# M4THYOU/TokenDagger

Hardware: AMD Instinct MI355X
Metric: GB/s raw text tokenized (Llama-4 vocab, 1024 MB corpus) (higher is better)
Workload: dtype u8

## Files before the change

### include/tokendagger_hip.h

```cpp
#ifndef TOKENDAGGER_HIP_H
#define TOKENDAGGER_HIP_H

#include <stdint.h>

#ifdef __cplusplus
extern "C" {
#endif

#define TD_OK 0
#define TD_E_INVALID 1
#define TD_E_PATTERN 2
#define TD_E_VOCAB 3
#define TD_E_UNKNOWN_BYTE 4
#define TD_E_CAPACITY 5
#define TD_E_SCRATCH 6
#define TD_E_HIP 7
#define TD_E_BAD_TOKEN 8
#define TD_E_SPECIAL 9

#define TD_MODE_ENCODE 0
#define TD_MODE_ORDINARY 1

typedef struct td_tokenizer td_tokenizer;

// ... 36 lines not shown
                                      const uint8_t* allowed_bytes, const int64_t* allowed_offsets, int64_t n_allowed,
                                      int32_t* out_tokens, int64_t out_capacity, int64_t* out_offsets, int64_t* n_tokens);

#define TD_INFO_N_PAIRS 1
#define TD_INFO_MERGE_CLOSED 2
#define TD_INFO_MAX_ID 3
#define TD_INFO_TILE_BYTES 4
#define TD_INFO_WORKSPACE_BYTES 5
#define TD_INFO_N_SPECIAL 6
#define TD_INFO_LONG_PIECES 7
#define TD_INFO_FAR_PIECES 8
#define TD_INFO_DEFERRED_TILES 9
#define TD_INFO_FLAGGED_TILES 10
#define TD_INFO_LB_TIMEOUTS 12
#define TD_INFO_REPEATS 13
#define TD_INFO_LISTED_PIECES 14
#define TD_INFO_CHAR_SEEDS 15
#define TD_INFO_SPARSE 16
#define TD_INFO_WS_FILLED_BYTES 17
#define TD_INFO_SMALL_ENCODES 18
#define TD_INFO_SMALL_ENCODE_HANDBACKS 19
#define TD_INFO_SMALL_DECODES 20
#define TD_INFO_SMALL_DECODE_HANDBACKS 21
#define TD_INFO_DIRECT_TILES 11
int64_t td_info(const td_tokenizer* t, int what);

int td_encode_device_with_special(td_tokenizer* t, const void* d_text, int64_t n_bytes, const void* d_doc_offsets, int64_t n_docs,
                                  const int32_t* allowed_ids, int64_t n_allowed, void* d_out_tokens, int64_t out_capacity,
                                  void* d_out_offsets, void* hip_stream);

#define TD_UNIT_BYTES 0
#define TD_UNIT_CHARS 1

int td_token_starts(td_tokenizer* t, const int32_t* tokens, int64_t n_tokens, const int64_t* tok_offsets, int64_t n_docs, int unit,
                    int64_t* out_starts);
int td_token_starts_device(td_tokenizer* t, const void* d_tokens, int64_t n_tokens, const void* d_tok_offsets, int64_t n_docs, int unit,
                           void* d_out_starts, void* hip_stream);

int td_encode_batch_with_starts(td_tokenizer* t, const uint8_t* text, const int64_t* doc_offsets, int64_t n_docs, int mode,
                                const uint8_t* allowed_bytes, const int64_t* allowed_offsets, int64_t n_allowed, int unit,
                                int32_t* out_tokens, int64_t out_capacity, int64_t* out_offsets, int64_t* out_starts, int64_t* n_tokens);

int td_encode_device_with_starts(td_tokenizer* t, const void* d_text, int64_t n_bytes, const void* d_doc_offsets, int64_t n_docs, int mode,
                                 int unit, void* d_out_tokens, int64_t out_capacity, void* d_out_offsets, void* d_out_starts,
                                 void* hip_stream);

// ... 425 lines not shown
```

### tokendagger_amd/capi.py

```python
from __future__ import annotations

import ctypes
from pathlib import Path

import numpy as np

_PKG = Path(__file__).resolve().parent
LIB_PATH = _PKG / "libtokendagger_hip.so"

TD_OK = 0
TD_E_CAPACITY = 5
TD_MODE_ENCODE = 0
TD_MODE_ORDINARY = 1
TD_E_INVALID = 1
TD_E_BAD_TOKEN = 8
TD_UNIT_BYTES, TD_UNIT_CHARS = 0, 1
TD_ROWS_CONCAT, TD_ROWS_PAD, TD_ROWS_BESTFIT, TD_ROWS_WINDOWS = 0, 1, 2, 3
TD_ROWS_DROP_LAST = 1
TD_ROWS_TRUNCATE = 2
TD_INFO_N_PAIRS, TD_INFO_MERGE_CLOSED, TD_INFO_MAX_ID, TD_INFO_TILE_BYTES = 1, 2, 3, 4
TD_INFO_WORKSPACE_BYTES, TD_INFO_N_SPECIAL, TD_INFO_LONG_PIECES, TD_INFO_FAR_PIECES = 5, 6, 7, 8
TD_OPT_LONG_POOL_BYTES = 1
TD_OPT_PROFILE = 2
TD_OPT_PIPE_CHUNK_BYTES = 3
# ... 4 lines not shown
TD_OPT_DEVICE_SPECIALS = 8
TD_OPT_DIRECT = 9
TD_OPT_PACK_SPLIT = 10
TD_OPT_DEDUPE = 11
TD_OPT_OVERLAP = 12
TD_OPT_GIANT_COOP_MIN = 13
TD_OPT_SPARSE = 14
TD_OPT_COUNTS_SEATS = 15
TD_OPT_COUNTS_FLUSH_TILES = 16
TD_COUNTS_ACCUMULATE = 1
TD_OPT_NGRAM_TAG_BITS = 17
TD_NGRAM_ACCUMULATE = 1
TD_NGRAM_MAX_LEN, TD_NGRAM_MAX_LENGTHS = 64, 8
TD_MINHASH_MAX_PERM = 1024
TD_NGRAM_INFO = {"patterns": 1, "distinct": 2, "lengths": 3, "max_len": 4, "slots": 5, "max_probe": 6, "device_bytes": 7}
TD_INFO_DEFERRED_TILES, TD_INFO_FLAGGED_TILES = 9, 10
TD_INFO_DIRECT_TILES = 11
TD_INFO_LB_TIMEOUTS = 12
TD_INFO_REPEATS, TD_INFO_LISTED_PIECES, TD_INFO_CHAR_SEEDS = 13, 14, 15
TD_INFO_SPARSE = 16
TD_OPT_WS_FILL = 18
TD_INFO_WS_FILLED_BYTES = 17
TD_INFO_SMALL_ENCODES, TD_INFO_SMALL_ENCODE_HANDBACKS, TD_INFO_SMALL_DECODES, TD_INFO_SMALL_DECODE_HANDBACKS = 18, 19, 20, 21

EXPORTS = [
    "td_create", "td_clone", "td_destroy", "td_last_error", "td_encode_batch", "td_encode_device", "td_reserve",
    "td_device_status", "td_decode_bytes", "td_encode_with_special", "td_info", "td_set_option",
    "td_special_count", "td_special_get", "td_profile_read",
    "td_vocab_create", "td_vocab_destroy", "td_vocab_error", "td_vocab_load_tiktoken", "td_vocab_load_hf_special",
    "td_vocab_load_tekken", "td_vocab_load_json", "td_vocab_set_pattern", "td_vocab_pattern", "td_vocab_arrays",
    "td_create_from_vocab", "td_token_bytes", "td_single_token", "td_decode_device", "td_decode_batch", "td_encode_batch_with_special",
    "td_encode_with_special_strs", "td_encode_batch_with_special_strs", "td_profile_read_ex", "td_profile_segment_name",
    "td_comm_unique_id", "td_comm_create", "td_comm_destroy", "td_comm_gather_counts", "td_comm_bases", "td_comm_gather_tokens",
    "td_comm_last_error", "td_encode_device_with_special", "td_token_starts", "td_token_starts_device", "td_encode_batch_with_starts",
    "td_encode_device_with_starts", "td_make_rows_device", "td_make_rows", "td_encode_batch_rows",
    "td_pack_plan", "td_pack_rows", "td_pack_rows_device", "td_encode_batch_pack_rows",
    "td_window_plan", "td_window_rows", "td_window_rows_device", "td_encode_batch_window_rows",
    "td_span_labels", "td_span_labels_device", "td_encode_batch_span_labels",
    "td_make_rows_labeled", "td_make_rows_labeled_device", "td_pack_rows_labeled", "td_pack_rows_labeled_device",
    "td_window_rows_labeled", "td_window_rows_labeled_device", "td_encode_batch_span_label_rows",
    "td_select_plan", "td_select_docs", "td_select_docs_device", "td_encode_batch_select",
    "td_join_plan", "td_join_fields", "td_join_fields_device", "td_encode_batch_join",
    "td_range_plan", "td_range_labels", "td_range_labels_device", "td_encode_batch_range_labels", "td_encode_batch_range_label_rows",
    "td_token_counts_host", "td_token_counts", "td_token_counts_device", "td_encode_batch_token_counts",
    "td_decode_rows_check", "td_decode_rows", "td_decode_rows_device",
    "td_ngram_set_create", "td_ngram_set_destroy", "td_ngram_set_info", "td_ngram_matches_host", "td_ngram_matches_device",
# ... 1967 lines not shown
```

### tokendagger_amd/csrc/td_api.cpp

```cpp
#include "td_counts_args.h"
#include "td_handle.h"
#include "td_regex.h"

static thread_local std::string g_create_err;
static thread_local std::string g_thread_err;
static thread_local const td_tokenizer* g_thread_err_owner = nullptr;

namespace td {

hipError_t make_stream(Stream& s) {
    hipStream_t h = nullptr;
    const hipError_t e = hipStreamCreateWithFlags(&h, hipStreamNonBlocking);
    if (e == hipSuccess) s = Stream(h);
    return e;
}
hipError_t make_event(Event& ev) {
    hipEvent_t h = nullptr;
    const hipError_t e = hipEventCreateWithFlags(&h, hipEventDisableTiming);
    if (e == hipSuccess) ev = Event(h);
    return e;
}
hipError_t make_pinned(PinnedBuf& b, size_t bytes) {
    void* p = nullptr;
    const hipError_t e = hipHostMalloc(&p, bytes, hipHostMallocDefault);
// ... 311 lines not shown
    a.dd_table = a.dedupe ? (unsigned long long*)t->dd_table.p : nullptr;
    a.dd_mask = a.dedupe ? dd_entries(t, n) - 1u : 0u;
    a.flagged_count = &ctl->flagged_count;
    a.rx = t->d_rx;
    a.rx_stage1 = t->d_rx_s1;
    a.rx_stage2 = t->d_rx_s2;
    a.gap_list = (int64_t*)t->gap_list.p;
    a.gap_cap = (uint32_t)std::min<size_t>(t->gap_list.cap / 4, 0x7FFFFFF0u);
    a.gapbits = (uint32_t*)t->gapbits.p;
    a.gx_chunk = gx_chunk_for(n);
    a.gx_exit = (int64_t*)t->gx_exit.p;
    a.gx_state = (uint32_t*)t->gx_state.p;
    a.gap_count = &ctl->gap_count;
    a.gx_prefix = t->gx_prefix_dev;
    a.flagged_list = (uint32_t*)t->flagged_list.p;
    a.deferred_list = (uint32_t*)t->deferred_list.p;
    a.deferred_count = &ctl->deferred_count;
    a.fused = t->opt.fused ? 1 : 0;
    a.pack_split = t->opt.pack_split ? 1 : 0;
    a.direct = (t->opt.direct && t->opt.fused && !t->sp_active && t->H.pattern_kind != PATTERN_GENERIC && d_out && !t->stop_after) ? 1 : 0;
    a.tile_state = (unsigned long long*)t->tile_state.p;
    a.slab = (uint32_t*)t->slab.p;
    a.direct_tiles = &ctl->direct_tiles;
    a.probe_deferred = 0;
    a.miss_cap = (uint32_t)((n_tiles + 1) * K_MISS_LISTED_MAX);
    a.chunk_pref = (int64_t*)t->chunk_pref.p;
    a.ctl_reset = &ctl->long_count;
    a.ctl_reset_words = (uint32_t)((sizeof(Ctl) - offsetof(Ctl, long_count)) / 4);
    a.out_tokens = (int32_t*)d_out;
    a.out_cap = d_out ? out_cap : 0;
    a.out_offsets = (int64_t*)d_out_offs;
    a.err = &ctl->err;
    a.err_pos = &ctl->err_pos;
    a.n_tiles = (int)n_tiles;
    a.n_stiles = (int)((n + KS_TILE - 1) / KS_TILE);
    a.pat_flags = pattern_flags(t->H.pattern_kind);
    a.use_fastpath = (mode == TD_MODE_ENCODE) || t->H.merge_closed;
    a.text_aligned = (((uintptr_t)d_text) & 15) == 0;
    a.stop_after = t->stop_after;
    if (t->sp_active) {
        a.sp.bytes = (const uint8_t*)t->sp_bytes.p;
        a.sp.off = (const uint32_t*)t->sp_off.p;
        a.sp.len = (const uint32_t*)t->sp_len.p;
        a.sp.id = (const int32_t*)t->sp_id.p;
        a.sp.parent = (const int32_t*)t->sp_parent.p;
        a.sp.first2 = (const uint32_t*)t->sp_first2.p;
// ... 82 lines not shown
            return "No value found for piece at byte offset " + std::to_string(pos) + ": byte sequence is not in the vocabulary";
        case TD_E_CAPACITY:
            return "output capacity too small: " + std::to_string(pos) + (rows_last ? " rows needed" : " tokens needed");
        case TD_E_BAD_TOKEN:
            return "Invalid token for decoding at index " + std::to_string(pos);
        case TD_E_SCRATCH:
            return "device scratch exhausted near byte offset " + std::to_string(pos) +
                   " (pieces above 64 bytes: raise TD_OPT_LONG_POOL_BYTES; allowed special tokens: more candidates than one per 32 bytes of the batch)";
    }
    return "device error " + std::to_string(code) + " at byte offset " + std::to_string(pos);
}

int td::absorb_ctl(td_tokenizer* t, Ctl c, hipStream_t stream, int64_t* err_pos) {
    int rc0;
    if (c.err == TD_E_BAD_TOKEN) c.err_pos = 0x7FFFFFFFFFFFFFFFll - c.err_pos;
    t->last_long = c.long_count;
    t->last_far = (int64_t)c.slow_count + c.far_tiles;
    t->last_giant = c.giant_count;
    t->seen_counters = true;
    t->last_deferred = c.deferred_count;
    t->last_flagged = c.flagged_count;
    t->last_direct = c.direct_tiles;
    t->last_timeouts = c.lb_timeouts;
    t->last_repeats = c.dd_stats[0];
    t->last_listed = c.dd_stats[1];
    if (err_pos) *err_pos = c.err_pos;
    if (c.err != 0) {
        if ((rc0 = zero_wait(t, t->ctl.p, sizeof(Ctl), stream))) return rc0;
        t->err = device_error_text(c.err, c.err_pos, t->rows_last);
        return c.err;
    }
    return TD_OK;
}

int td::device_status_locked(td_tokenizer* t, hipStream_t stream, int64_t* err_pos) {
    if (!t->ctl.p) { HIP_TRY(t, hipStreamSynchronize(stream)); return TD_OK; }
    int rc0 = own_streams(t);
    if (rc0) return rc0;
    static_assert(sizeof(Ctl) <= 256, "h_ctl");
    HIP_TRY(t, hipMemcpyAsync(t->h_ctl.p, t->ctl.p, sizeof(Ctl), hipMemcpyDeviceToHost, stream));
    HIP_TRY(t, hipStreamSynchronize(stream));
    if (!t->has_last || t->last_stream == stream) t->graveyard.clear();
    return absorb_ctl(t, *(const Ctl*)t->h_ctl.p, stream, err_pos);
}

namespace {
// ... 14 lines not shown
    t->s_h2d = std::move(h2d);
    return TD_OK;
}

int encode_batch_pipelined(td_tokenizer* t, const uint8_t* text, const int64_t* doc_offsets, int64_t n_docs, int mode,
                           int32_t* out_tokens, int64_t out_capacity, int64_t* out_offsets, int64_t* n_tokens) {
    int rc;
    if ((rc = pipe_init(t))) return rc;
    if (!t->pool_threads || t->pool_threads->size() != std::max(t->opt.pipe_threads - 1, 1)) t->pool_threads.reset(new CopyPool(std::max(t->opt.pipe_threads - 1, 1)));
    if ((rc = order_before(t, t->s_k))) return rc;
    const int64_t n_all = doc_offsets[n_docs] - doc_offsets[0];
    const int64_t chunk_bytes = std::min(t->opt.pipe_chunk_bytes, std::max<int64_t>(t->opt.pipe_chunk_bytes / 8, n_all / 6));
    std::vector<int64_t> cd{0};
    for (int64_t d = 0; d < n_docs;) {
        const int64_t lo = doc_offsets[d];
        int64_t e = d + 1;
        int64_t a = d + 1, b = n_docs;
        while (a < b) { const int64_t mid = (a + b + 1) >> 1; if (doc_offsets[mid] - lo <= chunk_bytes) a = mid; else b = mid - 1; }
        e = std::max(e, a);
        cd.push_back(e);
        d = e;
    }
    const int nchunks = (int)cd.size() - 1;
    t->last_direct = t->last_timeouts = 0;
    struct Pending { int64_t d0, d1, b0, nbytes, ntok; };
    std::vector<Pending> pend((size_t)nchunks);
    int64_t tok_base = 0;
    bool capacity_miss = false;
    int first_err = TD_OK;
    constexpr int NS = td_tokenizer::PIPE_SLOTS;
    const bool timing = getenv("TD_PIPE_TIMING") != nullptr;
    static const bool publish = !(getenv("TD_PIPE_PUBLISH") && atoi(getenv("TD_PIPE_PUBLISH")) == 0);
    static const int d2h_blocks = getenv("TD_PIPE_D2H_KERNEL") ? atoi(getenv("TD_PIPE_D2H_KERNEL")) : 32;
    double tm[6] = {0, 0, 0, 0, 0, 0};
    auto now = [] { return std::chrono::steady_clock::now(); };
    auto lap = [&](int k, std::chrono::steady_clock::time_point t0) { if (timing) tm[k] += std::chrono::duration<double, std::milli>(now() - t0).count(); };
    std::shared_ptr<CopyPool::Job> in_job[NS], out_job[NS];
    auto start_in = [&](int i) -> int {
        td_tokenizer::PipeSlot& sl = t->pipe[i % NS];
        const int64_t d0 = cd[(size_t)i], d1 = cd[(size_t)i + 1], b0 = doc_offsets[d0], nb = doc_offsets[d1] - b0;
        const auto t0 = now();
        int r;
        if ((r = pinned_ensure(t, sl.h_text, (size_t)nb + 64))) return r;
        in_job[i % NS] = t->pool_threads->copy(sl.h_text.p, text + b0, (size_t)nb);
        lap(5, t0);
        return TD_OK;
    };
// ... 22 lines not shown
        if ((r = encode_device_locked(t, sl.d_text.p, nb, sl.d_offs.p, nd, mode, sl.d_tok.p, std::max<int64_t>(nb, 1), sl.d_toff.p, t->s_k))) return r;
        if (publish) {
            HIP_TRY(t, launch_pipe_publish(t->ctl.p, (uint32_t)sizeof(Ctl), sl.h_ctl.p, (const int64_t*)sl.d_toff.p, nd + 1, (int64_t*)sl.h_offs.p, t->s_k));
        } else {
            HIP_TRY(t, hipMemcpyAsync(sl.h_ctl.p, t->ctl.p, sizeof(Ctl), hipMemcpyDeviceToHost, t->s_k));
            HIP_TRY(t, hipMemcpyAsync(sl.h_offs.p, sl.d_toff.p, (size_t)(nd + 1) * 8, hipMemcpyDeviceToHost, t->s_k));
        }
        HIP_TRY(t, hipEventRecord(sl.ev_off, t->s_k));
        lap(1, t0);
        return TD_OK;
    };
    auto fetch = [&](int i) -> int {
        td_tokenizer::PipeSlot& sl = t->pipe[i % NS];
        Pending& P = pend[(size_t)i];
        auto t0 = now();
        HIP_TRY(t, hipEventSynchronize(sl.ev_off));
        lap(2, t0);
        const int64_t nd = P.d1 - P.d0;
        const int64_t* to = (const int64_t*)sl.h_offs.p;
        const Ctl& c = *(const Ctl*)sl.h_ctl.p;
        P.ntok = to[nd];
        t->last_direct += c.direct_tiles;
        t->last_timeouts += c.lb_timeouts;
        if (c.err != 0 && first_err == TD_OK) {
            first_err = c.err;
            const long long pos = c.err_pos + (first_err == TD_E_UNKNOWN_BYTE || first_err == TD_E_SCRATCH ? P.b0 : 0);
            t->err = first_err == TD_E_UNKNOWN_BYTE ? device_error_text(first_err, pos, false)
                                                    : "device error " + std::to_string(first_err) + " near byte offset " + std::to_string(pos);
        }
        for (int64_t k = 0; k < nd; ++k) out_offsets[P.d0 + k] = tok_base + to[k];
        if (tok_base + P.ntok > out_capacity) capacity_miss = true;
        int r;
        t0 = now();
        if (out_job[i % NS]) { t->pool_threads->wait(out_job[i % NS]); out_job[i % NS].reset(); }
        lap(3, t0);
        if ((r = pinned_ensure(t, sl.h_tok, (size_t)std::max<int64_t>(P.ntok, 1) * 4))) return r;
        if (P.ntok > 0 && !capacity_miss && first_err == TD_OK)
        {
            if (d2h_blocks > 0) HIP_TRY(t, launch_pipe_copy_out(sl.d_tok.p, sl.h_tok.p, P.ntok, d2h_blocks, t->s_d2h));
            else HIP_TRY(t, hipMemcpyAsync(sl.h_tok.p, sl.d_tok.p, (size_t)P.ntok * 4, hipMemcpyDeviceToHost, t->s_d2h));
        }
        HIP_TRY(t, hipEventRecord(sl.ev_tok, t->s_d2h));
        const int64_t base = tok_base;
        tok_base += P.ntok;
        P.nbytes = base;
        return TD_OK;
// ... 382 lines not shown
    if (!t) return -1;
    switch (what) {
        case TD_INFO_N_PAIRS: return (int64_t)t->H.n_pairs;
        case TD_INFO_MERGE_CLOSED: return t->H.merge_closed ? 1 : 0;
        case TD_INFO_MAX_ID: return t->H.max_id;
        case TD_INFO_TILE_BYTES: return K_TILE;
        case TD_INFO_WORKSPACE_BYTES: return (int64_t)t->ws_bytes;
        case TD_INFO_N_SPECIAL: return (int64_t)t->H.special_ids.size();
        case TD_INFO_LONG_PIECES: return t->last_long;
        case TD_INFO_FAR_PIECES: return t->last_far;
        case TD_INFO_DEFERRED_TILES: return t->last_deferred;
        case TD_INFO_FLAGGED_TILES: return t->last_flagged;
        case TD_INFO_DIRECT_TILES: return t->last_direct;
        case TD_INFO_LB_TIMEOUTS: return t->last_timeouts;
        case TD_INFO_REPEATS: return t->last_repeats;
        case TD_INFO_LISTED_PIECES: return t->last_listed;
        case TD_INFO_CHAR_SEEDS: return (int64_t)t->H.n_char_seeds;
        case TD_INFO_SPARSE: return t->last_sparse ? 1 : 0;
        case TD_INFO_WS_FILLED_BYTES: return t->ws_filled;
        case TD_INFO_SMALL_ENCODES: return t->small_encodes;
        case TD_INFO_SMALL_ENCODE_HANDBACKS: return t->small_encode_handbacks;
        case TD_INFO_SMALL_DECODES: return t->small_decodes;
        case TD_INFO_SMALL_DECODE_HANDBACKS: return t->small_decode_handbacks;
    }
    return -1;
}

int td_set_option(td_tokenizer* t, int what, int64_t value) {
    if (!t) return TD_E_INVALID;
    std::lock_guard<std::mutex> g(t->mu);
    Options& o = t->opt;
    auto relaunch = [t] { drop_graph(t); t->has_last_key = false; return (int)TD_OK; };
    switch (what) {
        case TD_OPT_LONG_POOL_BYTES: if (value < (1 << 20)) break; o.pool_bytes_opt = value; return TD_OK;
#ifdef TD_ABLATE
        case 99: t->stop_after = (int)value; return TD_OK;
#endif
        case TD_OPT_FUSED: o.fused = value != 0; return TD_OK;
        case TD_OPT_DIRECT: o.direct = value != 0; return TD_OK;
        case TD_OPT_DEVICE_SPECIALS: o.device_specials = value != 0; return TD_OK;
        case TD_OPT_PACK_SPLIT: o.pack_split = value != 0; return relaunch();
        case TD_OPT_SPARSE: if (value < -1 || value > 1) break; o.sparse_opt = (int)value; return relaunch();
        case TD_OPT_OVERLAP: o.overlap = value != 0; return relaunch();
        case TD_OPT_GIANT_COOP_MIN: if (value < 1024) break; o.gp_coop_min = (uint32_t)std::min<int64_t>(value, 0x7FFFFFFF); return relaunch();
        case TD_OPT_DEDUPE: o.dedupe = value != 0; return relaunch();
        case TD_OPT_GRAPH: o.graphs = value != 0; return o.graphs ? (int)TD_OK : relaunch();
// ... 94 lines not shown
```

### tokendagger_amd/csrc/td_common.h

```cpp
#pragma once
#include <stdint.h>

#include "../../include/tokendagger_hip.h"

#if defined(__HIP__)
#define TD_HD __host__ __device__ inline __attribute__((always_inline))
#else
#define TD_HD inline
#endif

namespace td {

enum : uint32_t {
    C_OTHER = 0,
    C_APOS = 1,
    C_SLASH = 2,
    C_SP = 3,
    C_WS = 4,
    C_CRLF = 5,
    C_UP = 6,
    C_LW = 7,
    C_LB = 8,
    C_MK = 9,
    C_NUM = 10,
// ... 27 lines not shown
constexpr uint32_t TILE_DIRECT = 0x10000000u;
constexpr uint32_t TILE_MISS_LISTED = 0x20000000u;
constexpr int K_MISS_LISTED_MAX = 6;
constexpr int COLL_SUBS = 11;
constexpr int COLL_STRIDE = 32;
constexpr uint32_t TILE_OVF_SHIFT = 13;
constexpr int K_MISS_CLASSES = 5;
constexpr int ID_BITS = 21;
constexpr uint64_t PAIR_EMPTY = ~0ull;
constexpr uint64_t PAIR_KEY_MASK = (1ull << (2 * ID_BITS)) - 1;
constexpr uint64_t PAIR_FINAL = 1ull << 63;

struct PieceSlot {
    uint64_t key;
    uint32_t rank;
    uint32_t len;
};

struct Piece12Slot {
    uint32_t k0, k1, k2;
    uint32_t meta;
};
constexpr uint32_t P12_MAXLEN = 12;
TD_HD uint32_t p12_meta(uint32_t rank, uint32_t len) { return rank | (len << 24) | 0x80000000u; }

struct Tables {
    const uint8_t* ascii_cls;
    const uint16_t* ucls1;
    const uint8_t* ucls2;
    const int32_t* byte_id;
    const int32_t* byte_pair;
    const uint64_t* byte_pair_id;
    const PieceSlot* piece_slots;
    const uint64_t* pair_slots;
    const Piece12Slot* piece12_slots;
    const uint32_t* tok_off;
    const uint8_t* tok_bytes;
    uint32_t piece_mask;
    uint32_t pair_mask;
    int32_t max_id;
    int32_t pseudo_base;
    uint32_t max_token_len;
    uint32_t piece12_mask;
    uint32_t pat_flags;
    const uint64_t* cseed;
    const uint32_t* cseed_pm;
// ... 1094 lines not shown
```

### tokendagger_amd/csrc/td_handle.h

```cpp
#pragma once
#include <hip/hip_runtime.h>
#include <string.h>

#include <algorithm>
#include <atomic>
#include <chrono>
#include <condition_variable>
#include <deque>
#include <functional>
#include <memory>
#include <mutex>
#include <string>
#include <thread>
#include <vector>

#include "../../include/tokendagger_hip.h"
#include "td_kernels.h"
#include "td_rewrite_args.h"
#include "td_tables.h"

namespace td {
hipError_t launch_mid_done(const void* ctl, uint32_t ctl_bytes, void* h_ctl, unsigned long long* h_seq, unsigned long long seq, hipStream_t stream);
hipError_t launch_pipe_copy_out(const void* src, void* dst, int64_t n_words, int blocks, hipStream_t stream);
hipError_t launch_pipe_publish(const void* ctl, uint32_t ctl_bytes, void* h_ctl, const int64_t* d_toff, int64_t n_off, int64_t* h_toff, hipStream_t stream);
// ... 119 lines not shown
    int err;
    int pad;
    long long err_pos;
    uint32_t long_count;
    uint32_t slow_count;
    unsigned long long pool_used;
    uint32_t scan_done;
    uint32_t merge_next;
    uint32_t miss_count[6];
    uint32_t flagged_count;
    uint32_t gap_count;
    uint32_t deferred_count;
    uint32_t giant_count;
    uint32_t tile_draw;
    uint32_t direct_tiles;
    uint32_t lb_timeouts;
    uint32_t ovf_count;
    uint32_t dd_stats[2];
    uint32_t gp_ctl[4];
    uint32_t far_tiles;
    uint32_t ph_bar;
    uint32_t gs_done;
    uint32_t lp_next;
};
static_assert(K_MISS_CLASSES <= 6, "Ctl::miss_count");
constexpr size_t CTL_BYTES = 256;
static_assert(sizeof(Ctl) <= CTL_BYTES, "Ctl");

struct SharedTables {
    HostTables H;
    std::vector<void*> table_allocs;
    int device = 0;
    ~SharedTables() {
        if (table_allocs.empty()) return;
        DeviceGuard dg(device);
        for (void* p : table_allocs) (void)hipFree(p);
    }
};

struct RewriteBufs {
    DevBuf head, tiles, flags, counts, out, out_off;
};

struct Options {
    bool fused = true;
    bool graphs = false;
// ... 73 lines not shown
    int graph_failures = 0;
    GraphExec graph_exec;
    EncodeArgs graph_key, last_key;
    hipStream_t graph_stream = nullptr, last_key_stream = nullptr;
    bool has_last_key = false;
    std::vector<int32_t> sp_key;
    DevBuf sp_bytes, sp_off, sp_len, sp_id, sp_parent, sp_first2, sp_hit, sp_acc, sp_cpos, sp_clit, sp_ccount;
    uint32_t sp_n = 0, sp_maxlen = 0;
    bool sp_active = false;
    bool enc_keep_resident = false;
    bool enc_resident = false;
    const uint8_t* gx_prefix_host = nullptr;
    DevBuf gx_prefix;
    const uint8_t* gx_prefix_dev = nullptr;
    struct Ev3 {
        hipEvent_t e[TD_PROF_EVENTS] = {};
        Ev3() = default;
        Ev3(Ev3&& o) noexcept { std::swap(e, o.e); }
        Ev3& operator=(Ev3&& o) noexcept { std::swap(e, o.e); return *this; }
        ~Ev3() { for (hipEvent_t x : e) if (x) (void)hipEventDestroy(x); }
    };
    std::vector<Ev3> ev_pending, ev_free;
    int64_t last_repeats = 0, last_listed = 0;
    int64_t last_long = 0, last_far = 0, last_deferred = 0, last_flagged = 0, last_direct = 0, last_timeouts = 0;
    int64_t last_giant = 0;
    bool seen_counters = false;
    bool last_sparse = false;
    const RxProgram* d_rx = nullptr;
    const uint16_t* d_rx_s1 = nullptr;
    const uint8_t* d_rx_s2 = nullptr;
    size_t ws_bytes = 0;
    int64_t ws_filled = 0;
    Event last_done;
    hipStream_t last_stream = nullptr;
    bool has_last = false;
    std::vector<DevBuf> graveyard;
    struct PipeSlot {
        PinnedBuf h_text, h_offs, h_tok;
        DevBuf d_text, d_offs, d_tok, d_toff;
        Event ev_h2d, ev_k, ev_off, ev_tok;
        PinnedBuf h_ctl;
    };
    static constexpr int PIPE_SLOTS = 4;
    PipeSlot pipe[PIPE_SLOTS];
    Stream s_h2d, s_k, s_d2h;
    std::unique_ptr<CopyPool> pool_threads;
    PinnedBuf small_in, small_out;
// ... 88 lines not shown
```

### tokendagger_amd/csrc/td_kernels.h

```cpp
#pragma once
#include <hip/hip_runtime_api.h>
#include <stdint.h>

#include "td_common.h"
#include "td_special_dev.h"

namespace td {

struct RxProgram;

constexpr int TD_GP_SCRATCH_BYTES = 8192;
struct LongEntry {
    int64_t gs;
    uint32_t len;
    uint32_t ntok;
    uint64_t pool_off;
};

inline int gx_chunk_for(int64_t n) {
#ifdef TD_GX_CHUNK
    (void)n;
    return TD_GX_CHUNK;
#else
    int c = 64;
// ... 76 lines not shown
    int fused;
    int probe_deferred;
    SpecialTable sp;
    uint32_t* flagged_list;
    uint32_t* flagged_count;
    int64_t* chunk_pref;
    uint32_t* ctl_reset; uint32_t ctl_reset_words;
    int32_t* out_tokens;
    int64_t out_cap;
    int64_t* out_offsets;
    int* err;
    long long* err_pos;
    int n_tiles;
    int n_stiles;
    uint32_t pat_flags;
    int use_fastpath;
    int text_aligned;
    int stop_after;
    int pack_split;
    int direct;
    unsigned long long* tile_state;
    uint32_t* slab;
    uint32_t* direct_tiles;
};
constexpr unsigned long long TS_NONE = 0ull, TS_AGG = 1ull, TS_PREFIX = 2ull, TS_BROKEN = 3ull, TS_VALUE_MASK = (1ull << 62) - 1ull;
constexpr int SLAB_MAX_MISSES = 2 * 6;
constexpr int SLAB_META = 5136;
constexpr int SLAB_MIDS = SLAB_META + 2 * SLAB_MAX_MISSES;
constexpr int SLAB_WORDS = SLAB_MIDS + SLAB_MAX_MISSES * 64;
#ifndef TD_SLAB_RING
#define TD_SLAB_RING 3
#endif
constexpr int SLAB_RING = TD_SLAB_RING;

struct DecodeArgs {
    const Tables* Tp;
    const int32_t* tokens;
    int64_t n;
    uint32_t* local_off;
    int64_t* chunk_pref;
    uint32_t* scan_done;
    uint8_t* out;
    int64_t out_cap;
    int64_t* n_bytes;
    const int64_t* doc_tok_offsets;
    int64_t n_docs;
// ... 55 lines not shown
```

### tokendagger_amd/csrc/td_kernels.hip

```cpp
#include <hip/hip_runtime.h>
#include <stdlib.h>

#include "td_kernels.h"

namespace td {

#ifdef TD_ABLATE
#define TD_STOP(n) (a.stop_after == (n))
#else
#define TD_STOP(n) false
#endif

struct LdsSrc {
    const uint8_t* txt;
    const uint32_t* docw;
    int64_t lo, hi;
    __device__ __forceinline__ uint32_t byte(int64_t i) const { return txt[i]; }
    __device__ __forceinline__ bool doc(int64_t i) const { return (docw[i >> 5] >> (i & 31)) & 1u; }
};
struct GlobSrc {
    const uint8_t* text;
    const uint32_t* docbits;
    int64_t lo, hi;
    __device__ __forceinline__ uint32_t byte(int64_t i) const { return text[i]; }
// ... 632 lines not shown
    FreshArgs a{kernarg_args()};
    FreshTables T{(const __attribute__((address_space(4))) Tables*)a->Tp};
#define FZ_FRESH { a.refresh(); T.refresh(); }
#else
    const KeptArgs a{&a_kern};
    const Tables T_kept = uniform_tables(a->Tp);
    const KeptTables T{&T_kept};
#define FZ_FRESH
#endif
    for (int q = tid; q < 128; q += K_THREADS) s_lut[q] = (uint8_t)feature_of_class(T->ascii_cls[q]);
    if (tid < 16) s_fcls[tid] = (uint8_t)feature_of_class((uint32_t)tid);
    if (tid == 0) s_nonascii = 0;
    if (tid < 2) s_doc[K_WIN / 32 + tid] = 0;
    static_assert(K_WIN / 32 + 2 == CM_STRIDE, "the document bits cover the words the stored masks have");
    __shared__ __attribute__((aligned(16))) uint32_t s_kmask[FUSED ? (P12_MAXLEN + 1) * 4 : 4];
    __shared__ uint32_t s_wave[8];
    __shared__ uint32_t s_hflags[2], s_nrec[2], s_ncoldp;
    __shared__ uint32_t s_rec[2][K_MISS_LISTED_MAX];
    __shared__ unsigned long long s_pend[48];
    __shared__ uint32_t s_npend;
    __shared__ uint32_t s_flagl[32];
    __shared__ uint32_t s_nflagl;
    __shared__ uint32_t s_pd[DIRECT ? SLAB_RING : 1][PD_WORDS];
    __shared__ uint32_t s_stat[2];
    __shared__ unsigned long long s_lbv[4];
    __shared__ uint32_t s_lbs[4][3];
    __shared__ uint32_t s_brk;
    auto append_pending = [&](uint32_t npd) {
        const int ln = tid & 63;
        const bool have = (uint32_t)ln < npd;
        const unsigned long long rec = have ? s_pend[ln] : 0ull;
        const uint32_t c = mq_class((uint32_t)rec & 127u);
#pragma unroll
        for (uint32_t q = 0; q < (uint32_t)K_MISS_CLASSES; ++q) {
            const uint64_t b = __ballot(have && c == q);
            if (b) {
                const int leader = (int)td_ctz64(b);
                uint32_t at = 0;
                if (ln == leader) at = atomicAdd(&a->miss_count[q], (uint32_t)__popcll((unsigned long long)b));
                at = (uint32_t)__shfl((int)at, leader);
                if (have && c == q) a->miss_list[(size_t)q * a->miss_cap + at + (uint32_t)__popcll((unsigned long long)(b & ((1ull << ln) - 1ull)))] = rec;
            }
        }
    };
    if constexpr (FUSED) {
        if (tid < (int)(P12_MAXLEN + 1) * 4) {
            const int len = tid >> 2, w = tid & 3, nb = len - 4 * w;
            s_kmask[tid] = w == 3 || nb <= 0 ? 0u : nb >= 4 ? 0xFFFFFFFFu : (1u << (8 * nb)) - 1u;
        }
        if (tid == 0) { s_nflagl = 0; s_npend = 0; s_brk = 0; }
        if (DIRECT && tid < SLAB_RING * PD_WORDS) (&s_pd[0][0])[tid] = 0;
        if (tid < 2) s_stat[tid] = 0;
    }
    __syncthreads();

#ifndef TD_FUSED_NPRE
#define TD_FUSED_NPRE 0
#endif
    constexpr int NPF = (K_WIN / 16 + K_THREADS - 1) / K_THREADS;
    constexpr int NPRE = FUSED ? TD_FUSED_NPRE : NPF;
    uint4 pf[NPF];
    const int64_t nwords = (a->n + 31) >> 5;
    auto interior = [&](int64_t w0) { return a->text_aligned && w0 >= 0 && w0 + K_WIN <= a->n; };
    uint32_t pfd0 = 0, pfd1 = 0, pffd0 = 0xFFFFFFFFu, pffd1 = 0xFFFFFFFFu;
#ifdef TD_TEXT_L2_PREFETCH
    uint32_t pft = 0;
#endif
    static_assert(K_WIN / 32 <= 2 * K_THREADS, "two prefetched document words per lane cover the window");
    auto load_window = [&](int64_t w0) {
        {
            const int64_t gw0 = (w0 >> 5) + tid, gw1 = gw0 + K_THREADS;
            pfd0 = (gw0 >= 0 && gw0 < nwords) ? a->docbits[gw0] : 0u;
            pfd1 = (tid < K_WIN / 32 - K_THREADS && gw1 >= 0 && gw1 < nwords) ? a->docbits[gw1] : 0u;
            if (FUSED) {
                const int64_t t4 = (w0 + K_HL) / K_TILE;
// ... 678 lines not shown
                            const int i = (int)(il[q] >> 16);
                            const uint32_t len = il[q] & 0xFFFFu;
                            const u32x4 e = sl[q];
                            if (len <= P12_MAXLEN && fastpath &&
                                (e.w == 0u || (e.x == kk0[q] && e.y == kk1[q] && e.z == kk2[q] && (e.w >> 24) == (0x80u | len)))) {
                                const bool miss = e.w == 0u;
                                const uint32_t res = miss ? miss_marker(i, len) : (e.w & 0x1FFFFFu);
                                if (miss) {
                                    if (len == 1) raise(a, TD_E_UNKNOWN_BYTE, wg0 + i);
                                    note_miss(k, res);
                                }
                                (k < n0 ? dst0 : dst1)[k] = res;
                            } else {
                                const uint32_t j = atomicAdd(&s_ncoldp, 1u);
                                if (j < (uint32_t)FZ_CCAP) s_coldk[j] = (uint16_t)k;
                            }
                        }
                    }
                }
                __syncthreads();
                FZ_TICK(5)
                const uint32_t ncold = s_ncoldp;
                const bool cold_overflow = ncold > (uint32_t)FZ_CCAP;
                if (!cold_overflow) {
                    for (uint32_t c = tid; c < ncold; c += K_THREADS) {
                        const uint32_t k = s_coldk[c];
                        const int i = s_plist[k];
                        const uint32_t len = (uint32_t)s_plist[k + 1] - (uint32_t)i;
                        const uint32_t h = k >= n0 ? 1u : 0u;
                        uint32_t res = probe_piece_cold<true>(a, T, s_txt, T->byte_id, &s_hflags[h], wg0, i, len);
                        if ((res & 0xC0000000u) == TOK_MISS) { res = miss_marker(i, len); note_miss(k, res); }
                        (h ? dst1 : dst0)[k] = res;
                    }
                }
                __syncthreads();
                FZ_TICK(6)
                const bool resolved = cand && !cold_overflow && !(s_hflags[0] | s_hflags[1]) && s_nrec[0] <= (uint32_t)K_MISS_LISTED_MAX &&
                                      s_nrec[1] <= (uint32_t)K_MISS_LISTED_MAX;
                if (cold_overflow) {
                    if (tid == 0) {
                        const uint32_t at = atomicAdd(a->deferred_count, two ? 2u : 1u);
                        a->deferred_list[at] = (uint32_t)tile4;
                        if (two) a->deferred_list[at + 1] = (uint32_t)tile4 + 1u;
                        if (DIRECT) break_chain();
                    }
                } else if (resolved) {
                    FZ_TICK(12)
                    if (tid < 64) {
                        const uint32_t nr0 = s_nrec[0], nr1 = s_nrec[1], nm = nr0 + nr1;
                        uint32_t ext0 = 0, ext1 = 0;
                        if (nm) {
                            static_assert(2 * SLAB_MAX_MISSES * 4 * MG_UNIT * 4 <= FZ_R_COLDK, "keys + ids of the merged pieces fit the (dead) piece list");
                            uint32_t rec = 0, hh = 0;
                            if ((uint32_t)lane < nm) {
                                hh = (uint32_t)lane >= nr0 ? 1u : 0u;
                                rec = s_rec[hh][(uint32_t)lane - (hh ? nr0 : 0u)];
                            }
                            const uint32_t nt = fz_merge_piece(a->Tp, a->text, a->n, reinterpret_cast<uint32_t*>(s_R), slab, rec, hh, n0, tile_g0, a->err, a->err_pos);
// ... 88 lines not shown
                        }
                    }
                }
                FZ_TICK(9)
                }
            }
        }
        __syncthreads();
        ring = __builtin_amdgcn_readfirstlane(ring + 1 == SLAB_RING ? 0 : ring + 1);
        FZ_TICK(10)
#ifdef TD_FUSED_TIMING
        ++n_tiles_done;
#endif
    }
#ifdef TD_FUSED_TIMING
    if (FUSED && tid == 0 && (blockIdx.x % 211) == 0)
        printf("fused wg %d: %llu tiles, total %llu cycles | stage %llu masks %llu rules %llu heads %llu | list %llu probe %llu cold %llu bookkeeping %llu lookback %llu docs %llu tail %llu place %llu | t12 %llu t13 %llu\n",
               (int)blockIdx.x, n_tiles_done, (unsigned long long)(__builtin_readcyclecounter() - t_total0), tt[0], tt[1], tt[2], tt[3], tt[4], tt[5], tt[6], tt[7],
               tt[8], tt[9], tt[10], tt[11], tt[12], tt[13]);
#endif
    if constexpr (FUSED) {
        if (DIRECT && tid == 0 && s_stat[0]) atomicAdd(a->direct_tiles, s_stat[0]);
        if (DIRECT && tid == 0 && s_stat[1]) atomicAdd(a->direct_tiles + 1, s_stat[1]);
        if (tid < 64) append_pending(s_npend);
        if (tid == 0 && s_nflagl) {
            const uint32_t nf = s_nflagl, at = atomicAdd(a->flagged_count, nf);
            for (uint32_t q = 0; q < nf; ++q) a->flagged_list[at + q] = s_flagl[q];
        }
    }
}

struct WaveMaskP {
    const Tables& T;
    const uint8_t* text;
    const uint32_t* docbits;
    int64_t n, g;
    int o, lim;
    int lane;
    __device__ __forceinline__ uint32_t cf_at(int64_t pos) const {
        if (pos >= n) return F_DOC;
        GlobSrc src;
        src.text = text; src.docbits = docbits; src.lo = 0; src.hi = n;
        uint32_t v = classify_at(T, src, pos);
        if (src.doc(pos)) v |= F_DOC;
        return v;
    }
// ... 161 lines not shown
    }
}
__global__ __launch_bounds__(256) void td_split_far_tiles(const EncodeArgs a) { far_tiles_body(a, blockIdx.x, gridDim.x); }

__device__ __forceinline__ void probe_tiles_body(const EncodeArgs& a, const uint32_t bid, const uint32_t nb) {
    __shared__ __attribute__((aligned(16))) uint8_t s_txt[K_BWIN + 16];
    __shared__ uint32_t s_start[K_BWIN / 32 + 3];
    __shared__ __attribute__((aligned(16))) uint16_t s_plist[K_TILE + 8];
    uint32_t* const s_off = reinterpret_cast<uint32_t*>(s_plist);
    uint16_t* const s_valid = s_plist + 2 * K_THREADS;
    __shared__ int32_t s_byteid[256];
    __shared__ __attribute__((aligned(16))) uint32_t s_kmask[(P12_MAXLEN + 1) * 4];
    __shared__ uint32_t s_wave[8];
    __shared__ long long s_ext_end;
    __shared__ uint32_t s_flags;
    __shared__ uint32_t s_nrec;
    __shared__ uint32_t s_rec[K_MISS_LISTED_MAX];
    __shared__ unsigned long long s_pend[64];
    __shared__ uint32_t s_npend;
    __shared__ uint32_t s_flagl[32];
    __shared__ uint32_t s_nflagl;
    __shared__ uint32_t s_ncold;
    __shared__ uint16_t s_coldk[K_THREADS];

    const int tid = threadIdx.x;
    const Tables T = uniform_tables(a.Tp);
    for (int q = tid; q < 256; q += K_THREADS) s_byteid[q] = T.byte_id[q];
    if (tid == 0) { s_npend = 0; s_nflagl = 0; }
    if (tid < (int)(P12_MAXLEN + 1) * 4) {
        const int len = tid >> 2, w = tid & 3, nb = len - 4 * w;
        s_kmask[tid] = w == 3 || nb <= 0 ? 0u : nb >= 4 ? 0xFFFFFFFFu : (1u << (8 * nb)) - 1u;
    }

    uint4 pf0 = make_uint4(0, 0, 0, 0), pf1 = pf0;
    uint32_t pfs = 0;
    const uint32_t list_max = TD_STOP(70) ? 0u : (uint32_t)K_MISS_LISTED_MAX;
    auto append_pending = [&](uint32_t np) {
        const int ln = tid & 63;
        const bool have = (uint32_t)ln < np;
        const unsigned long long rec = have ? s_pend[ln] : 0ull;
        const uint32_t c = mq_class((uint32_t)rec & 127u);
#pragma unroll
        for (uint32_t q = 0; q < (uint32_t)K_MISS_CLASSES; ++q) {
            const uint64_t b = __ballot(have && c == q);
            if (b) {
                const int leader = (int)td_ctz64(b);
                uint32_t at = 0;
                if (ln == leader) at = atomicAdd(&a.miss_count[q], (uint32_t)__popcll((unsigned long long)b));
                at = (uint32_t)__shfl((int)at, leader);
                if (have && c == q) a.miss_list[(size_t)q * a.miss_cap + at + (uint32_t)__popcll((unsigned long long)(b & ((1ull << ln) - 1ull)))] = rec;
            }
// ... 107 lines not shown
            uint32_t res;
            if (len <= P12_MAXLEN && a.use_fastpath && !last_ext && (sl.w == 0u || (sl.x == k0 && sl.y == k1 && sl.z == k2 && (sl.w >> 24) == (0x80u | len)))) {
                const bool miss = sl.w == 0u;
                res = miss ? (TOK_MISS | ((uint32_t)i << 7) | len) : (sl.w & 0x1FFFFFu);
                if (miss) {
                    if (len == 1) raise(a, TD_E_UNKNOWN_BYTE, wg0 + i);
                    note_miss(k, res);
                }
            } else {
                const uint32_t j = atomicAdd(&s_ncold, 1u);
                if (j < (uint32_t)K_THREADS) { s_coldk[j] = (uint16_t)k; continue; }
                if (last_ext) {
                    const long long l = ext_end - (wg0 + i);
                    len = l > 0x7FFFFFFFll ? 0xFFFFFFFFu : (uint32_t)l;
                }
                res = probe_piece_cold<false>(a, T, s_txt, s_byteid, &s_flags, wg0, i, len);
                if ((res & 0xC0000000u) == TOK_MISS) note_miss(k, res);
            }
            dst[k] = res;
        }
        __syncthreads();
        {
            const uint32_t nc = s_ncold < (uint32_t)K_THREADS ? s_ncold : (uint32_t)K_THREADS;
            if ((uint32_t)tid < nc) {
                const uint32_t k = s_coldk[tid];
                const int i = s_plist[k];
                uint32_t len = (uint32_t)s_plist[k + 1] - (uint32_t)i;
                if (ext_end && k == np_total - 1) {
                    const long long l = ext_end - (wg0 + i);
                    len = l > 0x7FFFFFFFll ? 0xFFFFFFFFu : (uint32_t)l;
                }
                const uint32_t res = probe_piece_cold<false>(a, T, s_txt, s_byteid, &s_flags, wg0, i, len);
                if ((res & 0xC0000000u) == TOK_MISS) note_miss(k, res);
                dst[k] = res;
            }
        }
        __syncthreads();
        if (TD_STOP(3)) continue;
        s_off[tid] = pbase;
        s_valid[tid] = (uint16_t)smask0;
        {
            const uint32_t nr = s_nrec, np0 = s_npend;
            if (tid < 64) {
                const bool listed = nr && nr <= list_max;
                if (listed && (uint32_t)tid < nr) s_pend[np0 + tid] = ((unsigned long long)(uint32_t)tile << 32) | s_rec[tid];
                const uint32_t np1 = listed ? np0 + nr : np0;
// ... 18 lines not shown
                    const uint32_t at = atomicAdd(a.flagged_count, 32u);
                    for (uint32_t q = 0; q < 32u; ++q) a.flagged_list[at + q] = s_flagl[q];
                    nf = 0;
                }
                s_nflagl = nf;
            }
            else if (nr) fl |= TILE_MISS_LISTED;
            a.tile_count[tile] = np_total | fl;
        }
        __syncthreads();
        {
            const int64_t tile_end_g = tile_g0 + tile_hi;
            const int64_t fd = (int64_t)a.tile_first_doc[tile];
            for (int64_t d = fd + tid; d < a.n_docs; d += K_THREADS) {
                const int64_t p = a.doc_offsets[d];
                if (p >= tile_end_g) break;
                const int lp = (int)(p - tile_g0);
                a.doc_slot[d] = s_off[lp >> 4] + __popc((uint32_t)s_valid[lp >> 4] & ((1u << (lp & 15)) - 1u));
            }
        }
        __syncthreads();
    }
    if (tid < 64) append_pending(s_npend);
    if (tid == 0 && s_nflagl) {
        const uint32_t nf = s_nflagl, at = atomicAdd(a.flagged_count, nf);
        for (uint32_t q = 0; q < nf; ++q) a.flagged_list[at + q] = s_flagl[q];
    }
}
__global__ __launch_bounds__(K_THREADS, TD_PROBE_MIN_WAVES) void td_probe_tiles(const EncodeArgs a) { probe_tiles_body(a, blockIdx.x, gridDim.x); }

constexpr int DD_BUF = 512 + 64;
__device__ __forceinline__ void dd_chunk(const uint8_t* text, int64_t n_text, int64_t g, uint32_t left, uint32_t (&w)[4]) {
    uint32_t t[5];
    load_piece_window(text, n_text, g, t);
#pragma unroll
    for (int i = 0; i < 4; ++i) {
        const int32_t l = (int32_t)left - 4 * i;
        w[i] = l >= 4 ? t[i] : l <= 0 ? 0u : (t[i] & ((1u << (8 * l)) - 1u));
    }
}
__device__ __forceinline__ uint32_t dd_mix(uint32_t h, uint32_t w) {
    uint32_t k = w * 0xCC9E2D51u;
    k = (k << 15) | (k >> 17);
    h ^= k * 0x1B873593u;
    return ((h << 13) | (h >> 19)) * 5u + 0xE6546B64u;
}
// ... 3149 lines not shown
```

### tokendagger_amd/csrc/td_tables.cpp

```cpp
#include "td_tables.h"
#include <cstdio>
#include <cstdlib>
#include "td_regex.h"

#include <string.h>

#include <algorithm>
#include <map>

#include "generated/unicode_classes.inc"

namespace td {

static const char kO200k[] =
    "[^\\r\\n\\p{L}\\p{N}]?[\\p{Lu}\\p{Lt}\\p{Lm}\\p{Lo}\\p{M}]*[\\p{Ll}\\p{Lm}\\p{Lo}\\p{M}]+(?i:'s|'t|'re|'ve|'m|'ll|'d)?"
    "|[^\\r\\n\\p{L}\\p{N}]?[\\p{Lu}\\p{Lt}\\p{Lm}\\p{Lo}\\p{M}]+[\\p{Ll}\\p{Lm}\\p{Lo}\\p{M}]*(?i:'s|'t|'re|'ve|'m|'ll|'d)?"
    "|\\p{N}{1,3}| ?[^\\s\\p{L}\\p{N}]+[\\r\\n/]*|\\s*[\\r\\n]+|\\s+(?!\\S)|\\s+";

static const char kTekken[] =
    "[^\\r\\n\\p{L}\\p{N}]?[\\p{Lu}\\p{Lt}\\p{Lm}\\p{Lo}\\p{M}]*[\\p{Ll}\\p{Lm}\\p{Lo}\\p{M}]+"
    "|[^\\r\\n\\p{L}\\p{N}]?[\\p{Lu}\\p{Lt}\\p{Lm}\\p{Lo}\\p{M}]+[\\p{Ll}\\p{Lm}\\p{Lo}\\p{M}]*"
    "|\\p{N}| ?[^\\s\\p{L}\\p{N}]+[\\r\\n/]*|\\s*[\\r\\n]+|\\s+(?!\\S)|\\s+";

static const char kCl100k[] =
// ... 321 lines not shown
        uint32_t h = hash_piece(key, len) & H.piece_mask;
        for (;;) {
            PieceSlot& s = H.piece_slots[h];
            if (s.len == 0) { s.key = key; s.rank = (uint32_t)ranks[v]; s.len = len; break; }
            if (s.key == key && s.len == len &&
                (len <= 8 || memcmp(&H.tok_bytes[H.tok_off[s.rank]], p, len) == 0)) {
                err = "duplicate token bytes in vocabulary";
                return TD_E_VOCAB;
            }
            h = (h + 1) & H.piece_mask;
        }
        if (len == 1) H.byte_id[p[0]] = ranks[v];
        if (len == 2) H.byte_pair[((uint32_t)p[0] << 8) | p[1]] = ranks[v];
    }

    H.byte_pair_id.resize(65536);
    for (uint32_t q = 0; q < 65536; ++q) H.byte_pair_id[q] = (uint64_t)(uint32_t)H.byte_pair[q] | ((uint64_t)(uint32_t)H.byte_id[q >> 8] << 32);

    {
        std::vector<int64_t> order;
        for (int64_t v = 0; v < n_vocab; ++v)
            if (token_offsets[v + 1] - token_offsets[v] <= (int64_t)P12_MAXLEN) order.push_back(v);
        std::sort(order.begin(), order.end(), [&](int64_t x, int64_t y) { return ranks[x] < ranks[y]; });
        const uint32_t cap12 = pow2_at_least((uint64_t)order.size() * 2 + 2);
        H.piece12_mask = cap12 - 1;
        H.piece12_slots.assign(cap12, Piece12Slot{0, 0, 0, 0});
        for (int64_t v : order) {
            const uint32_t len = (uint32_t)(token_offsets[v + 1] - token_offsets[v]);
            const uint8_t* p = token_bytes + token_offsets[v];
            uint32_t k[3] = {0, 0, 0};
            for (uint32_t i = 0; i < len; ++i) k[i >> 2] |= (uint32_t)p[i] << (8 * (i & 3));
            uint32_t h = hash_piece12(k[0], k[1], k[2], len) & H.piece12_mask;
            while (H.piece12_slots[h].meta != 0) h = (h + 1) & H.piece12_mask;
            H.piece12_slots[h] = Piece12Slot{k[0], k[1], k[2], p12_meta((uint32_t)ranks[v], len)};
        }
    }

    Tables T = H.view();
    auto id_of = [&](const uint8_t* p, uint32_t len) -> int32_t {
        if (len == 1) return H.byte_id[p[0]];
        return piece_lookup(T, piece_key_host(p, len), len, [p](uint32_t i) { return (uint32_t)p[i]; });
    };
    std::vector<std::pair<uint64_t, uint32_t>> pairs;
    pairs.reserve((size_t)n_vocab * 3);
    for (int64_t v = 0; v < n_vocab; ++v) {
        const uint8_t* p = token_bytes + token_offsets[v];
        const uint32_t len = (uint32_t)(token_offsets[v + 1] - token_offsets[v]);
        for (uint32_t k = 1; k < len; ++k) {
            const int32_t l = id_of(p, k);
            if (l == NO_RANK) continue;
            const int32_t r = id_of(p + k, len - k);
            if (r == NO_RANK) continue;
            pairs.emplace_back(((uint64_t)(uint32_t)l << ID_BITS) | (uint32_t)r, (uint32_t)ranks[v]);
        }
    }
    H.n_pairs = pairs.size();
    for (uint32_t qcap = pow2_at_least((uint64_t)pairs.size() * 2 + 2);; qcap <<= 1) {
// ... 58 lines not shown
```

Measured before the change: 488.8.

## Make exact-key piece table sparser and direct-mapped, skip empty cold-pass barrier

The exact-key table for pieces of up to 12 bytes now gets a compile-time number of slots per token (default 4, up from 2). Each token is inserted only into its home slot with no linear probing, so colliding tokens are left out and must be resolved by the slower cold probe path. The fused kernel also skips the cold-resolution loop and its __syncthreads when a tile has no cold pieces. New counters for cold pieces are added and exposed through td_info. The trade is a larger table and more cold fallbacks on collisions, in exchange for shorter, more predictable hot-path probes.

```diff
diff --git a/include/tokendagger_hip.h b/include/tokendagger_hip.h
--- a/include/tokendagger_hip.h
+++ b/include/tokendagger_hip.h
@@ -82,6 +82,7 @@
 #define TD_INFO_SMALL_ENCODE_HANDBACKS 19
 #define TD_INFO_SMALL_DECODES 20
 #define TD_INFO_SMALL_DECODE_HANDBACKS 21
+#define TD_INFO_COLD_PIECES 22
 #define TD_INFO_DIRECT_TILES 11
 int64_t td_info(const td_tokenizer* t, int what);
 
diff --git a/tokendagger_amd/capi.py b/tokendagger_amd/capi.py
--- a/tokendagger_amd/capi.py
+++ b/tokendagger_amd/capi.py
@@ -50,6 +50,7 @@
 TD_OPT_WS_FILL = 18
 TD_INFO_WS_FILLED_BYTES = 17
 TD_INFO_SMALL_ENCODES, TD_INFO_SMALL_ENCODE_HANDBACKS, TD_INFO_SMALL_DECODES, TD_INFO_SMALL_DECODE_HANDBACKS = 18, 19, 20, 21
+TD_INFO_COLD_PIECES = 22
 
 EXPORTS = [
     "td_create", "td_clone", "td_destroy", "td_last_error", "td_encode_batch", "td_encode_device", "td_reserve",
diff --git a/tokendagger_amd/csrc/td_api.cpp b/tokendagger_amd/csrc/td_api.cpp
--- a/tokendagger_amd/csrc/td_api.cpp
+++ b/tokendagger_amd/csrc/td_api.cpp
@@ -357,6 +357,7 @@
     a.tile_state = (unsigned long long*)t->tile_state.p;
     a.slab = (uint32_t*)t->slab.p;
     a.direct_tiles = &ctl->direct_tiles;
+    a.cold_pieces = &ctl->cold_pieces;
     a.probe_deferred = 0;
     a.miss_cap = (uint32_t)((n_tiles + 1) * K_MISS_LISTED_MAX);
     a.chunk_pref = (int64_t*)t->chunk_pref.p;
@@ -485,6 +486,7 @@
     t->last_flagged = c.flagged_count;
     t->last_direct = c.direct_tiles;
     t->last_timeouts = c.lb_timeouts;
+    t->last_cold = c.cold_pieces;
     t->last_repeats = c.dd_stats[0];
     t->last_listed = c.dd_stats[1];
     if (err_pos) *err_pos = c.err_pos;
@@ -545,7 +547,7 @@
         d = e;
     }
     const int nchunks = (int)cd.size() - 1;
-    t->last_direct = t->last_timeouts = 0;
+    t->last_direct = t->last_timeouts = t->last_cold = 0;
     struct Pending { int64_t d0, d1, b0, nbytes, ntok; };
     std::vector<Pending> pend((size_t)nchunks);
     int64_t tok_base = 0;
@@ -614,6 +616,7 @@
         P.ntok = to[nd];
         t->last_direct += c.direct_tiles;
         t->last_timeouts += c.lb_timeouts;
+        t->last_cold += c.cold_pieces;
         if (c.err != 0 && first_err == TD_OK) {
             first_err = c.err;
             const long long pos = c.err_pos + (first_err == TD_E_UNKNOWN_BYTE || first_err == TD_E_SCRATCH ? P.b0 : 0);
@@ -1042,6 +1045,7 @@
         case TD_INFO_SMALL_ENCODE_HANDBACKS: return t->small_encode_handbacks;
         case TD_INFO_SMALL_DECODES: return t->small_decodes;
         case TD_INFO_SMALL_DECODE_HANDBACKS: return t->small_decode_handbacks;
+        case TD_INFO_COLD_PIECES: return t->last_cold;
     }
     return -1;
 }
diff --git a/tokendagger_amd/csrc/td_common.h b/tokendagger_amd/csrc/td_common.h
--- a/tokendagger_amd/csrc/td_common.h
+++ b/tokendagger_amd/csrc/td_common.h
@@ -73,6 +73,10 @@
     uint32_t meta;
 };
 constexpr uint32_t P12_MAXLEN = 12;
+#ifndef TD_P12_SLOTS_PER_TOKEN
+#define TD_P12_SLOTS_PER_TOKEN 4
+#endif
+static_assert(TD_P12_SLOTS_PER_TOKEN >= 1 && TD_P12_SLOTS_PER_TOKEN <= 64, "TD_P12_SLOTS_PER_TOKEN: slots per token of the exact-key table");
 TD_HD uint32_t p12_meta(uint32_t rank, uint32_t len) { return rank | (len << 24) | 0x80000000u; }
 
 struct Tables {
diff --git a/tokendagger_amd/csrc/td_handle.h b/tokendagger_amd/csrc/td_handle.h
--- a/tokendagger_amd/csrc/td_handle.h
+++ b/tokendagger_amd/csrc/td_handle.h
@@ -165,6 +165,7 @@
     uint32_t ph_bar;
     uint32_t gs_done;
     uint32_t lp_next;
+    uint32_t cold_pieces;
 };
 static_assert(K_MISS_CLASSES <= 6, "Ctl::miss_count");
 constexpr size_t CTL_BYTES = 256;
@@ -284,7 +285,7 @@
     };
     std::vector<Ev3> ev_pending, ev_free;
     int64_t last_repeats = 0, last_listed = 0;
-    int64_t last_long = 0, last_far = 0, last_deferred = 0, last_flagged = 0, last_direct = 0, last_timeouts = 0;
+    int64_t last_long = 0, last_far = 0, last_deferred = 0, last_flagged = 0, last_direct = 0, last_timeouts = 0, last_cold = 0;
     int64_t last_giant = 0;
     bool seen_counters = false;
     bool last_sparse = false;
diff --git a/tokendagger_amd/csrc/td_kernels.h b/tokendagger_amd/csrc/td_kernels.h
--- a/tokendagger_amd/csrc/td_kernels.h
+++ b/tokendagger_amd/csrc/td_kernels.h
@@ -122,6 +122,7 @@
     unsigned long long* tile_state;
     uint32_t* slab;
     uint32_t* direct_tiles;
+    uint32_t* cold_pieces;
 };
 constexpr unsigned long long TS_NONE = 0ull, TS_AGG = 1ull, TS_PREFIX = 2ull, TS_BROKEN = 3ull, TS_VALUE_MASK = (1ull << 62) - 1ull;
 constexpr int SLAB_MAX_MISSES = 2 * 6;
diff --git a/tokendagger_amd/csrc/td_kernels.hip b/tokendagger_amd/csrc/td_kernels.hip
--- a/tokendagger_amd/csrc/td_kernels.hip
+++ b/tokendagger_amd/csrc/td_kernels.hip
@@ -678,7 +678,7 @@
     __shared__ uint32_t s_flagl[32];
     __shared__ uint32_t s_nflagl;
     __shared__ uint32_t s_pd[DIRECT ? SLAB_RING : 1][PD_WORDS];
-    __shared__ uint32_t s_stat[2];
+    __shared__ uint32_t s_stat[3];
     __shared__ unsigned long long s_lbv[4];
     __shared__ uint32_t s_lbs[4][3];
     __shared__ uint32_t s_brk;
@@ -706,7 +706,7 @@
         }
         if (tid == 0) { s_nflagl = 0; s_npend = 0; s_brk = 0; }
         if (DIRECT && tid < SLAB_RING * PD_WORDS) (&s_pd[0][0])[tid] = 0;
-        if (tid < 2) s_stat[tid] = 0;
+        if (tid < 3) s_stat[tid] = 0;
     }
     __syncthreads();
 
@@ -1431,18 +1431,21 @@
                 FZ_TICK(5)
                 const uint32_t ncold = s_ncoldp;
                 const bool cold_overflow = ncold > (uint32_t)FZ_CCAP;
-                if (!cold_overflow) {
-                    for (uint32_t c = tid; c < ncold; c += K_THREADS) {
-                        const uint32_t k = s_coldk[c];
-                        const int i = s_plist[k];
-                        const uint32_t len = (uint32_t)s_plist[k + 1] - (uint32_t)i;
-                        const uint32_t h = k >= n0 ? 1u : 0u;
-                        uint32_t res = probe_piece_cold<true>(a, T, s_txt, T->byte_id, &s_hflags[h], wg0, i, len);
-                        if ((res & 0xC0000000u) == TOK_MISS) { res = miss_marker(i, len); note_miss(k, res); }
-                        (h ? dst1 : dst0)[k] = res;
+                if (ncold) {
+                    if (!cold_overflow) {
+                        if (tid == 0) s_stat[2] += ncold;
+                        for (uint32_t c = tid; c < ncold; c += K_THREADS) {
+                            const uint32_t k = s_coldk[c];
+                            const int i = s_plist[k];
+                            const uint32_t len = (uint32_t)s_plist[k + 1] - (uint32_t)i;
+                            const uint32_t h = k >= n0 ? 1u : 0u;
+                            uint32_t res = probe_piece_cold<true>(a, T, s_txt, T->byte_id, &s_hflags[h], wg0, i, len);
+                            if ((res & 0xC0000000u) == TOK_MISS) { res = miss_marker(i, len); note_miss(k, res); }
+                            (h ? dst1 : dst0)[k] = res;
+                        }
                     }
-                }
-                __syncthreads();
+                    __syncthreads();
+                }
                 FZ_TICK(6)
                 const bool resolved = cand && !cold_overflow && !(s_hflags[0] | s_hflags[1]) && s_nrec[0] <= (uint32_t)K_MISS_LISTED_MAX &&
                                       s_nrec[1] <= (uint32_t)K_MISS_LISTED_MAX;
@@ -1577,6 +1580,7 @@
     if constexpr (FUSED) {
         if (DIRECT && tid == 0 && s_stat[0]) atomicAdd(a->direct_tiles, s_stat[0]);
         if (DIRECT && tid == 0 && s_stat[1]) atomicAdd(a->direct_tiles + 1, s_stat[1]);
+        if (tid == 0 && s_stat[2]) atomicAdd(a->cold_pieces, s_stat[2]);
         if (tid < 64) append_pending(s_npend);
         if (tid == 0 && s_nflagl) {
             const uint32_t nf = s_nflagl, at = atomicAdd(a->flagged_count, nf);
@@ -1784,11 +1788,12 @@
     __shared__ uint32_t s_nflagl;
     __shared__ uint32_t s_ncold;
     __shared__ uint16_t s_coldk[K_THREADS];
+    __shared__ uint32_t s_coldsum;
 
     const int tid = threadIdx.x;
     const Tables T = uniform_tables(a.Tp);
     for (int q = tid; q < 256; q += K_THREADS) s_byteid[q] = T.byte_id[q];
-    if (tid == 0) { s_npend = 0; s_nflagl = 0; }
+    if (tid == 0) { s_npend = 0; s_nflagl = 0; s_coldsum = 0; }
     if (tid < (int)(P12_MAXLEN + 1) * 4) {
         const int len = tid >> 2, w = tid & 3, nb = len - 4 * w;
         s_kmask[tid] = w == 3 || nb <= 0 ? 0u : nb >= 4 ? 0xFFFFFFFFu : (1u << (8 * nb)) - 1u;
@@ -1942,6 +1947,7 @@
         __syncthreads();
         {
             const uint32_t nc = s_ncold < (uint32_t)K_THREADS ? s_ncold : (uint32_t)K_THREADS;
+            if (tid == 0) s_coldsum += s_ncold;
             if ((uint32_t)tid < nc) {
                 const uint32_t k = s_coldk[tid];
                 const int i = s_plist[k];
@@ -2006,6 +2012,7 @@
         __syncthreads();
     }
     if (tid < 64) append_pending(s_npend);
+    if (tid == 0 && s_coldsum) atomicAdd(a.cold_pieces, s_coldsum);
     if (tid == 0 && s_nflagl) {
         const uint32_t nf = s_nflagl, at = atomicAdd(a.flagged_count, nf);
         for (uint32_t q = 0; q < nf; ++q) a.flagged_list[at + q] = s_flagl[q];
diff --git a/tokendagger_amd/csrc/td_tables.cpp b/tokendagger_amd/csrc/td_tables.cpp
--- a/tokendagger_amd/csrc/td_tables.cpp
+++ b/tokendagger_amd/csrc/td_tables.cpp
@@ -367,7 +367,7 @@
         for (int64_t v = 0; v < n_vocab; ++v)
             if (token_offsets[v + 1] - token_offsets[v] <= (int64_t)P12_MAXLEN) order.push_back(v);
         std::sort(order.begin(), order.end(), [&](int64_t x, int64_t y) { return ranks[x] < ranks[y]; });
-        const uint32_t cap12 = pow2_at_least((uint64_t)order.size() * 2 + 2);
+        const uint32_t cap12 = pow2_at_least((uint64_t)order.size() * TD_P12_SLOTS_PER_TOKEN + 2);
         H.piece12_mask = cap12 - 1;
         H.piece12_slots.assign(cap12, Piece12Slot{0, 0, 0, 0});
         for (int64_t v : order) {
@@ -375,9 +375,8 @@
             const uint8_t* p = token_bytes + token_offsets[v];
             uint32_t k[3] = {0, 0, 0};
             for (uint32_t i = 0; i < len; ++i) k[i >> 2] |= (uint32_t)p[i] << (8 * (i & 3));
-            uint32_t h = hash_piece12(k[0], k[1], k[2], len) & H.piece12_mask;
-            while (H.piece12_slots[h].meta != 0) h = (h + 1) & H.piece12_mask;
-            H.piece12_slots[h] = Piece12Slot{k[0], k[1], k[2], p12_meta((uint32_t)ranks[v], len)};
+            Piece12Slot& home = H.piece12_slots[hash_piece12(k[0], k[1], k[2], len) & H.piece12_mask];
+            if (home.meta == 0) home = Piece12Slot{k[0], k[1], k[2], p12_meta((uint32_t)ranks[v], len)};
         }
     }
 
```

Result: slower. 481.7 (-1.5%).
